# qq456cvb/CPPF2

Hardware: AMD Instinct MI355X
Metric: scenes/sec (1/2/4/8 GPU) at 4096 pts x 20k tuples; 5deg5cm match vs ref (higher is better)
Workload: dtype f32

## Files before the change

cppf2_amd/csrc/cppf_vote.hip:

```cpp
#include "cppf_common.h"
#include <mutex>

#define VC_THREADS 1024
#ifndef VC_SLAB_CELLS
#define VC_SLAB_CELLS 36864
#endif
#define VC_ARG_BLOCKS 32
#ifndef VC_MAX_LDS_ROTS
#define VC_MAX_LDS_ROTS 512
#endif
#define VC_TAB_LEN (2 * VC_MAX_LDS_ROTS + 4)
#define VC_LDS_WORDS (VC_SLAB_CELLS + 2 * VC_TAB_LEN + (VC_THREADS / 64) * 64)
#ifndef VC_MIN_SLAB_CELLS
#define VC_MIN_SLAB_CELLS 8192
#endif
#ifndef VC_MIN_WAVES
#define VC_MIN_WAVES 4
#endif
#define VC_FRAME_FLOATS 12
#define VC_WT_SCALE 256.0f
#ifndef VC_QUANTUM
#define VC_QUANTUM 4
#endif
#ifndef VC_ARC_MARGIN
// ... 546 lines not shown
    __syncthreads();
    const int item = s_item;
    if (item >= count) break;
    const uint32_t e = list[item / parts];
    const int b = (int)(e & 0xffffu), s = (int)(e >> 16);
    const CppfSceneGrid g = grids[b];
    vote_slab_item<true, WEIGHTED>(slab, tag, b, s, slab_cells, item % parts, parts, g, g.ncell, fr, total, tup_off, res, num_rots,
                                   cos_tab, sin_tab, grid, grid_off, cells_cap, slab_best, s_max, 1, part, tickets);
  }
}

__global__ __launch_bounds__(256) void vote_center_global_kernel(
    const float* __restrict__ pts, const int32_t* __restrict__ pt_off, const int32_t* __restrict__ idx, int k,
    const int32_t* __restrict__ tup_off, const float* __restrict__ tr, const float* __restrict__ vote_wt, float res,
    int num_rots, const float* __restrict__ cos_tab, const float* __restrict__ sin_tab,
    const CppfSceneGrid* __restrict__ grids, uint32_t* __restrict__ grid, const int64_t* __restrict__ grid_off,
    int64_t cells_cap) {
  const int b = blockIdx.y;
  const CppfSceneGrid g = grids[b];
  if ((int64_t)g.ncell > cells_cap || g.ncell <= 0) return;
  const float* p = pts + 3 * (int64_t)pt_off[b];
  const int t0 = tup_off[b], nt = tup_off[b + 1] - t0;
  uint32_t* gb = grid + (grid_off ? grid_off[b] : (int64_t)b * cells_cap);
  for (int t = blockIdx.x * blockDim.x + threadIdx.x; t < nt; t += gridDim.x * blockDim.x) {
    const int64_t row = (int64_t)(t0 + t);
    const VoteSetup v = vote_setup(p, idx[row * k], idx[row * k + 1], tr[row * 2], tr[row * 2 + 1], res);
    if (!v.ok) continue;
    const uint32_t wv = vote_weight(vote_wt, row);
    for (int r = 0; r < num_rots; ++r) {
      const int lin = vote_cell(v.cx, v.cy, v.cz, v.xx, v.xy, v.xz, v.yx, v.yy, v.yz, cos_tab[r], sin_tab[r],
                                g.c0[0], g.c0[1], g.c0[2], res, g.g[0], g.g[1], g.g[2]);
      if (lin >= 0) atomicAdd(&gb[lin], wv);
    }
  }
}

__global__ __launch_bounds__(256) void grid_argmax_partial_kernel(const uint32_t* __restrict__ grid,
                                                                  const int64_t* __restrict__ grid_off,
                                                                  int64_t cells_cap,
                                                                  const CppfSceneGrid* __restrict__ grids,
                                                                  SlabBest* __restrict__ partial, int s_max) {
  const int b = blockIdx.y;
  const int G = ((int64_t)grids[b].ncell <= cells_cap) ? grids[b].ncell : 0;
  const uint32_t* gb = grid + (grid_off ? grid_off[b] : (int64_t)b * cells_cap);
  const int per = (G + gridDim.x - 1) / gridDim.x;
  const int lo = blockIdx.x * per, hi = min(G, lo + per);
  uint32_t bv = 0;
  int64_t bi = INT64_MAX;
  for (int i = lo + threadIdx.x; i < hi; i += blockDim.x) argmax_combine(bv, bi, gb[i], (int64_t)i);
  wave_argmax(bv, bi);
  __shared__ uint32_t s_v[4];
  __shared__ int64_t s_i[4];
  if (wave_lane() == 0) { s_v[threadIdx.x >> 6] = bv; s_i[threadIdx.x >> 6] = bi; }
  __syncthreads();
  if (threadIdx.x == 0) {
    for (int w = 1; w < 4; ++w) argmax_combine(bv, bi, s_v[w], s_i[w]);
    SlabBest o; o.idx = bi; o.val = bv; o.pad = 0;
    partial[(int64_t)b * s_max + blockIdx.x] = o;
  }
}

__global__ __launch_bounds__(64) void grid_argmax_final_kernel(const SlabBest* __restrict__ partial, int s_max,
                                                               int fixed_parts, const int* __restrict__ ctl,
                                                               const CppfSceneGrid* __restrict__ grids,
                                                               int64_t cells_cap, double res,
                                                               int64_t* __restrict__ out_argmax,
                                                               uint32_t* __restrict__ out_peak,
                                                               double* __restrict__ out_world) {
  const int b = blockIdx.x;
  const CppfSceneGrid g = grids[b];
  const int G = ((int64_t)g.ncell <= cells_cap) ? g.ncell : 0;
  const int slab_cells = ctl ? ctl[3] : VC_SLAB_CELLS;
  const int parts = fixed_parts > 0 ? fixed_parts : (G + slab_cells - 1) / slab_cells;
  uint32_t bv = 0;
  int64_t bi = INT64_MAX;
  for (int i = threadIdx.x; i < parts; i += 64) {
    const SlabBest sb = partial[(int64_t)b * s_max + i];
    argmax_combine(bv, bi, sb.val, sb.idx);
  }
  wave_argmax(bv, bi);
  if (threadIdx.x == 0) {
    if (bi == INT64_MAX) bi = 0;
    out_argmax[b] = bi;
    if (out_peak) out_peak[b] = ((int64_t)g.ncell > cells_cap) ? 0xFFFFFFFFu : bv;
    if (out_world) {
      const int64_t gyz = (int64_t)g.g[1] * g.g[2];
      const int64_t ix = gyz > 0 ? bi / gyz : 0;
      const int64_t rem = gyz > 0 ? bi - ix * gyz : 0;
      const int64_t iy = g.g[2] > 0 ? rem / g.g[2] : 0;
      const int64_t iz = g.g[2] > 0 ? rem - iy * g.g[2] : 0;
      out_world[3 * b + 0] = (double)g.c0[0] + (double)ix * res;
      out_world[3 * b + 1] = (double)g.c0[1] + (double)iy * res;
      out_world[3 * b + 2] = (double)g.c0[2] + (double)iz * res;
    }
  }
}

__global__ __launch_bounds__(256) void grid_zero_kernel(uint32_t* __restrict__ grid,
                                                        const int64_t* __restrict__ grid_off, int64_t cells_cap,
                                                        const CppfSceneGrid* __restrict__ grids) {
  const int b = blockIdx.y;
  const int G = ((int64_t)grids[b].ncell <= cells_cap) ? grids[b].ncell : 0;
  uint32_t* gb = grid + (grid_off ? grid_off[b] : (int64_t)b * cells_cap);
  for (int i = blockIdx.x * blockDim.x + threadIdx.x; i < G; i += gridDim.x * blockDim.x) gb[i] = 0u;
}

static inline int64_t align_up(int64_t x, int64_t a) { return (x + a - 1) / a * a; }

static inline int vc_parts(int64_t cells_cap) {
  int64_t s_max = (cells_cap + VC_SLAB_CELLS - 1) / VC_SLAB_CELLS;
  if (s_max < VC_ARG_BLOCKS) s_max = VC_ARG_BLOCKS;
  return (int)s_max;
}

extern "C" int64_t cppf_vote_center_workspace_bytes(int B, int64_t cells_cap, int64_t total_tuples) {
  if (B <= 0 || cells_cap <= 0 || total_tuples < 0) return 0;
  return align_up((int64_t)B * vc_parts(cells_cap) * (int64_t)sizeof(SlabBest), 256) +
         align_up((int64_t)B * vc_parts(cells_cap) * 4 + 256, 256) + align_up((int64_t)B * vc_parts(cells_cap) * 4, 256) +
         align_up((int64_t)B * cells_cap * 4, 256) + align_up(total_tuples * VC_FRAME_FLOATS * 4, 256);
}

extern "C" int cppf_vote_center(int B, const float* pts, const int32_t* pt_off, const int32_t* idx, int k,
                                const int32_t* tup_off, int max_t, int64_t total_tuples, const float* tr,
                                const float* vote_wt, double res, int num_rots, const float* cos_tab, const float* sin_tab, const CppfSceneGrid* grids,
                                uint32_t* grid, const int64_t* grid_off, int64_t cells_cap, int mode,
                                void* workspace, int64_t workspace_bytes, int64_t* out_argmax, uint32_t* out_peak,
                                double* out_world, void* stream) {
  CPPF_CHECK_ARG(B > 0 && pts && pt_off && idx && tup_off && tr && cos_tab && sin_tab && grids && out_argmax);
  CPPF_CHECK_ARG(k >= 2 && num_rots > 0 && res > 0.0 && cells_cap > 0 && cells_cap <= 0x7fffffffLL);
  CPPF_CHECK_ARG(total_tuples >= 0 && max_t >= 0 && (int64_t)max_t <= total_tuples);
  CPPF_CHECK_ARG(workspace && workspace_bytes >= cppf_vote_center_workspace_bytes(B, cells_cap, total_tuples));
  CPPF_CHECK_ARG(grid == nullptr || grid_off != nullptr);
  hipStream_t st = (hipStream_t)stream;
  const int s_max_parts = vc_parts(cells_cap);
  SlabBest* best = (SlabBest*)workspace;
  char* wsp = (char*)workspace + align_up((int64_t)B * s_max_parts * sizeof(SlabBest), 256);
  int* ws_ctl = (int*)wsp;
  uint32_t* ws_list = (uint32_t*)(wsp + 256);
  wsp += align_up((int64_t)B * s_max_parts * 4 + 256, 256);
  int* ws_tickets = (int*)wsp;
  wsp += align_up((int64_t)B * s_max_parts * 4, 256);
  uint32_t* ws_grid = (uint32_t*)wsp;
  float* frames = (float*)(wsp + align_up((int64_t)B * cells_cap * 4, 256));
  const int s_max = (int)((cells_cap + VC_SLAB_CELLS - 1) / VC_SLAB_CELLS);
  const bool frames_only = (mode & CPPF_VC_FRAMES_ONLY) != 0, frames_ready = (mode & CPPF_VC_FRAMES_READY) != 0;
  const int mode_bits = mode;
  mode &= 0xff;
  if (mode == 0) mode = (s_max <= 64) ? 1 : 2;
  int exhaustive = 0;
  if (mode == 3) { mode = 1; exhaustive = 1; }
  const float res32 = (float)res;
  if (max_t <= 0) mode = 2;

  if (mode == 1) {
    int P = 1;
    const int64_t wgs = (int64_t)B * s_max;
    if (wgs < 256) {
      P = (int)((256 + wgs - 1) / wgs);
      const int pmax = (max_t + VC_THREADS - 1) / VC_THREADS;
      if (P > pmax) P = pmax;
      if (P < 1) P = 1;
    }
    const int lds_bytes = VC_LDS_WORDS * 4;
    static std::mutex cu_mutex;
    static int cu_count[64] = {0};
    int dev = 0;
    CPPF_HIP(hipGetDevice(&dev));
    const int dslot = dev & 63;
    {
      std::lock_guard<std::mutex> lock(cu_mutex);
      if (cu_count[dslot] == 0) {
        hipDeviceProp_t prop;
        CPPF_HIP(hipGetDeviceProperties(&prop, dev));
        const void* fns[] = {(const void*)vote_center_slab_kernel<true, false>, (const void*)vote_center_slab_kernel<true, true>,
                             (const void*)vote_center_slab_kernel<false, false>, (const void*)vote_center_slab_kernel<false, true>,
                             (const void*)vote_center_persist_kernel<false>, (const void*)vote_center_persist_kernel<true>};
        for (const void* f : fns) CPPF_HIP(hipFuncSetAttribute(f, hipFuncAttributeMaxDynamicSharedMemorySize, lds_bytes));
        cu_count[dslot] = prop.multiProcessorCount > 0 ? prop.multiProcessorCount : 256;
      }
    }
    const int num_cus = cu_count[dslot];
    const bool arcs = (exhaustive == 0) && s_max > 1 && num_rots <= VC_MAX_LDS_ROTS && num_rots >= 8;
    const bool persist = arcs && B <= 0xffff && s_max <= 0xffff && (mode_bits & 0x800) == 0;
    uint32_t* g_use = grid;
    const int64_t* goff_use = grid_off;
    if (P > 1 && !persist) {
      if (!g_use) { g_use = ws_grid; goff_use = nullptr; }
      hipLaunchKernelGGL(grid_zero_kernel, dim3(64, B), dim3(256), 0, st, g_use, goff_use, cells_cap, grids);
      CPPF_LAUNCH_CHECK();
    }
    if (persist) {
      const int pmax_t = (max_t + VC_THREADS - 1) / VC_THREADS;
      const int max_parts = (B <= 48) ? (pmax_t < 64 ? (pmax_t < 1 ? 1 : pmax_t) : 64) : 1;
      if (!frames_ready) {
        hipLaunchKernelGGL(vote_frames_kernel, dim3((max_t + 255) / 256, B), dim3(256), 0, st, pts, pt_off, idx, k,
                           tup_off, tr, vote_wt, res32, num_rots, total_tuples, frames);
        hipLaunchKernelGGL(vote_worklist_kernel, dim3(1), dim3(1024), 0, st, grids, B, cells_cap, s_max_parts, max_parts,
                           2 * num_cus, ws_list, ws_ctl);
        if (max_parts > 1) {
          hipLaunchKernelGGL(grid_zero_kernel, dim3(64, B), dim3(256), 0, st, ws_grid, (const int64_t*)nullptr, cells_cap,
                             grids);
          CPPF_HIP(hipMemsetAsync(ws_tickets, 0, (size_t)B * s_max_parts * 4, st));
        }
        CPPF_LAUNCH_CHECK();
      }
      if (frames_only) return CPPF_OK;
      if (vote_wt)
        hipLaunchKernelGGL(vote_center_persist_kernel<true>, dim3(num_cus), dim3(VC_THREADS), lds_bytes, st, frames,
                           total_tuples, tup_off, res32, num_rots, cos_tab, sin_tab, grids, grid, grid_off, cells_cap, best,
                           s_max_parts, ws_list, ws_ctl, max_parts > 1 ? ws_grid : (uint32_t*)nullptr, ws_tickets);
      else
        hipLaunchKernelGGL(vote_center_persist_kernel<false>, dim3(num_cus), dim3(VC_THREADS), lds_bytes, st, frames,
                           total_tuples, tup_off, res32, num_rots, cos_tab, sin_tab, grids, grid, grid_off, cells_cap, best,
                           s_max_parts, ws_list, ws_ctl, max_parts > 1 ? ws_grid : (uint32_t*)nullptr, ws_tickets);
      CPPF_LAUNCH_CHECK();
      hipLaunchKernelGGL(grid_argmax_final_kernel, dim3(B), dim3(64), 0, st, best, s_max_parts, 0, (const int*)ws_ctl, grids, cells_cap, res,
                         out_argmax, out_peak, out_world);
      CPPF_LAUNCH_CHECK();
      return CPPF_OK;
    }
    if (!frames_ready) {
      hipLaunchKernelGGL(vote_frames_kernel, dim3((max_t + 255) / 256, B), dim3(256), 0, st, pts, pt_off, idx, k,
                         tup_off, tr, vote_wt, res32, num_rots, total_tuples, frames);
      CPPF_LAUNCH_CHECK();
    }
    if (frames_only) return CPPF_OK;
    {
      const dim3 gr(B, P, s_max), bl(VC_THREADS);
#define VC_LAUNCH_SLAB(A, W)                                                                                          \
  hipLaunchKernelGGL((vote_center_slab_kernel<A, W>), gr, bl, lds_bytes, st, frames, total_tuples, tup_off, res32,       \
                     num_rots, cos_tab, sin_tab, grids, g_use, goff_use, cells_cap, best, s_max_parts, P)
      if (arcs) { if (vote_wt) VC_LAUNCH_SLAB(true, true); else VC_LAUNCH_SLAB(true, false); }
      else      { if (vote_wt) VC_LAUNCH_SLAB(false, true); else VC_LAUNCH_SLAB(false, false); }
#undef VC_LAUNCH_SLAB
    }
    CPPF_LAUNCH_CHECK();
    if (P == 1) {
      hipLaunchKernelGGL(grid_argmax_final_kernel, dim3(B), dim3(64), 0, st, best, s_max_parts, 0, (const int*)nullptr, grids, cells_cap,
                         res, out_argmax, out_peak, out_world);
    } else {
      hipLaunchKernelGGL(grid_argmax_partial_kernel, dim3(VC_ARG_BLOCKS, B), dim3(256), 0, st, g_use, goff_use,
                         cells_cap, grids, best, s_max_parts);
      hipLaunchKernelGGL(grid_argmax_final_kernel, dim3(B), dim3(64), 0, st, best, s_max_parts, VC_ARG_BLOCKS, (const int*)nullptr, grids,
                         cells_cap, res, out_argmax, out_peak, out_world);
    }
    CPPF_LAUNCH_CHECK();
    return CPPF_OK;
  }
  if (mode == 2) {
    uint32_t* g_use = grid ? grid : ws_grid;
    const int64_t* goff_use = grid ? grid_off : nullptr;
    hipLaunchKernelGGL(grid_zero_kernel, dim3(64, B), dim3(256), 0, st, g_use, goff_use, cells_cap, grids);
    CPPF_LAUNCH_CHECK();
    if (max_t > 0) {
      hipLaunchKernelGGL(vote_center_global_kernel, dim3((max_t + 255) / 256, B), dim3(256), 0, st, pts, pt_off, idx,
                         k, tup_off, tr, vote_wt, res32, num_rots, cos_tab, sin_tab, grids, g_use, goff_use, cells_cap);
      CPPF_LAUNCH_CHECK();
    }
    hipLaunchKernelGGL(grid_argmax_partial_kernel, dim3(VC_ARG_BLOCKS, B), dim3(256), 0, st, g_use, goff_use,
                       cells_cap, grids, best, s_max_parts);
    hipLaunchKernelGGL(grid_argmax_final_kernel, dim3(B), dim3(64), 0, st, best, s_max_parts, VC_ARG_BLOCKS, (const int*)nullptr, grids,
                       cells_cap, res, out_argmax, out_peak, out_world);
    CPPF_LAUNCH_CHECK();
    return CPPF_OK;
  }
  snprintf(g_cppf_err, sizeof(g_cppf_err), "cppf_vote_center: unknown mode %d", mode);
  return CPPF_EINVAL;
}

#ifndef BV_THREADS
#define BV_THREADS 1024
#endif

__device__ __forceinline__ int block_scan_flag(bool flag, int* s_wave, int* total) {
  const unsigned long long m = __ballot(flag);
  const int lane = wave_lane(), w = threadIdx.x >> 6;
  const int within = __popcll(m & ((1ull << lane) - 1ull));
  if (lane == 0) s_wave[w] = __popcll(m);
  __syncthreads();
  int base = 0, tot = 0;
  for (int i = 0; i < BV_THREADS / 64; ++i) {
    const int c = s_wave[i];
    if (i < w) base += c;
    tot += c;
  }
  __syncthreads();
  *total = tot;
  return base + within;
}

template <typename KeyFn>
__device__ uint32_t radix_select_keys(KeyFn key, int n, int kth, uint32_t* s_hist , int* s_misc ,
                                      int* n_le) {
  uint32_t prefix = 0;
  int remaining = kth;
  int below = 0;
  const int shifts[3] = {21, 10, 0};
  const int widths[3] = {11, 11, 10};
  uint32_t mask_fixed = 0;
  for (int pass = 0; pass < 3; ++pass) {
    const int sh = shifts[pass], nbins = 1 << widths[pass];
    for (int i = threadIdx.x; i < nbins; i += blockDim.x) s_hist[i] = 0;
    __syncthreads();
    for (int i = threadIdx.x; i < n; i += blockDim.x) {
      const uint32_t bits = key(i);
      if ((bits & mask_fixed) == prefix) atomicAdd(&s_hist[(bits >> sh) & (nbins - 1)], 1u);
    }
    __syncthreads();
    if (threadIdx.x < 64) {
      const int per = nbins / 64;
      uint32_t sum = 0;
      for (int j = 0; j < per; ++j) sum += s_hist[threadIdx.x * per + j];
      uint32_t incl = sum;
#pragma unroll
      for (int off = 1; off < 64; off <<= 1) {
        const uint32_t o = __shfl_up(incl, off);
        if ((int)threadIdx.x >= off) incl += o;
      }
      const uint32_t excl = incl - sum;
      if ((uint32_t)remaining >= excl && (uint32_t)remaining < incl) {
        uint32_t run = excl;
        for (int j = 0; j < per; ++j) {
          const uint32_t c = s_hist[threadIdx.x * per + j];
          if ((uint32_t)remaining < run + c) {
            s_misc[0] = threadIdx.x * per + j;
            s_misc[1] = (int)run;
            s_misc[2] = (int)c;
            break;
          }
          run += c;
        }
      }
    }
    __syncthreads();
    const int bin = s_misc[0];
    below += s_misc[1];
    remaining -= s_misc[1];
    prefix |= ((uint32_t)bin) << sh;
    mask_fixed |= ((uint32_t)(nbins - 1)) << sh;
    if (pass == 2) *n_le = below + s_misc[2];
    __syncthreads();
  }
  return prefix;
}

__device__ uint32_t radix_select(const float* __restrict__ v, int n, int kth, uint32_t* s_hist, int* s_misc,
                                 int* n_le) {
  return radix_select_keys([v](int i) { return __float_as_uint(v[i]); }, n, kth, s_hist, s_misc, n_le);
}

__device__ __forceinline__ uint32_t float_key(float f) {
  const uint32_t u = __float_as_uint(f);
  return (u & 0x80000000u) ? ~u : (u | 0x80000000u);
}
__device__ __forceinline__ float key_float(uint32_t k) {
  return __uint_as_float((k & 0x80000000u) ? (k & 0x7fffffffu) : ~k);
}

__global__ __launch_bounds__(256) void backvote_errs_kernel(const float* __restrict__ pts,
                                                            const int32_t* __restrict__ pt_off,
                                                            const int32_t* __restrict__ idx, int k,
                                                            const int32_t* __restrict__ tup_off,
                                                            const float* __restrict__ tr,
                                                            const double* __restrict__ centers, Axes9 axes,
                                                            float* __restrict__ errs) {
  const int b = blockIdx.y;
  const float* p = pts + 3 * (int64_t)pt_off[b];
  const int t0 = tup_off[b], nt = tup_off[b + 1] - t0;
  const double cx = centers[3 * b], cy = centers[3 * b + 1], cz = centers[3 * b + 2];
  for (int t = blockIdx.x * 256 + threadIdx.x; t < nt; t += gridDim.x * 256) {
    const int64_t row = (int64_t)(t0 + t);
    const float* a = p + 3 * (int64_t)idx[row * k];
    const float* bb = p + 3 * (int64_t)idx[row * k + 1];
    float tb[2];
    target_pair(a[0], a[1], a[2], bb[0], bb[1], bb[2], cx, cy, cz, axes.a, tb, nullptr);
    const float d0 = tr[row * 2] - tb[0], d1 = tr[row * 2 + 1] - tb[1];
    errs[row] = __builtin_sqrtf(d0 * d0 + d1 * d1);
  }
}

__global__ __launch_bounds__(BV_THREADS) void backvote_kernel(
    const float* __restrict__ pts, const int32_t* __restrict__ pt_off, const int32_t* __restrict__ idx, int k,
    const int32_t* __restrict__ tup_off, const float* __restrict__ tr, const double* __restrict__ centers,
    Axes9 axes, const int32_t* __restrict__ kidx, const float* __restrict__ gammas, double margin, int num_rots,
    uint8_t* __restrict__ mask, int32_t* __restrict__ kept_tuple, int32_t* __restrict__ kept_count,
    double* __restrict__ kept_wt, int32_t* __restrict__ kept_row0, float* __restrict__ errs,
    float* __restrict__ thr_out, int32_t* __restrict__ hits) {
  __shared__ uint32_t s_hist[2048];
  __shared__ int s_misc[4];
  __shared__ int s_wave[BV_THREADS / 64];
  __shared__ float s_f[BV_THREADS / 64];
  const int b = blockIdx.x;
  const int p0 = pt_off[b];
  const float* p = pts + 3 * (int64_t)p0;
  const int t0 = tup_off[b], nt = tup_off[b + 1] - t0;
  float* e = errs + t0;
  if (nt <= 0) {
    if (threadIdx.x == 0) { kept_count[b] = 0; if (thr_out) thr_out[b] = NAN; }
    return;
  }
  int kq = kidx[b];
  if (kq > nt - 1) kq = nt - 1;
  const float gamma = gammas[b];
  int n_le = 0;
  const uint32_t bits_lo = radix_select(e, nt, kq, s_hist, s_misc, &n_le);
  const float v_lo = __uint_as_float(bits_lo);
  float v_hi = v_lo;
  if (kq + 1 <= nt - 1 && kq + 1 >= n_le) {
    uint32_t mn = 0xffffffffu;
    for (int i = threadIdx.x; i < nt; i += BV_THREADS) {
      const uint32_t bits = __float_as_uint(e[i]);
      if (bits > bits_lo && bits < mn) mn = bits;
    }
#pragma unroll
    for (int off = 32; off > 0; off >>= 1) mn = min(mn, (uint32_t)__shfl_xor((int)mn, off));
    if (wave_lane() == 0) s_hist[threadIdx.x >> 6] = mn;
    __syncthreads();
    if (threadIdx.x == 0) {
      for (int w = 1; w < BV_THREADS / 64; ++w) mn = min(mn, s_hist[w]);
      s_hist[64] = mn;
    }
    __syncthreads();
    v_hi = __uint_as_float(s_hist[64]);
    __syncthreads();
  }
  const float diff = v_hi - v_lo;
  float thr = v_lo + diff * gamma;
  if (gamma >= 0.5f) thr = v_hi - diff * (1.0f - gamma);
  if (threadIdx.x == 0 && thr_out) thr_out[b] = thr;
  int kept = 0;
  for (int base = 0; base < nt; base += BV_THREADS) {
    const int t = base + threadIdx.x;
    const bool keep = (t < nt) && (e[t] < thr);
    if (t < nt) mask[t0 + t] = keep ? 1 : 0;
    int tot;
    const int pos = block_scan_flag(keep, s_wave, &tot);
    if (keep) kept_tuple[t0 + kept + pos] = t;
    kept += tot;
  }
  if (threadIdx.x == 0) kept_count[b] = kept;
  __syncthreads();
  int32_t* h = hits + p0;
  for (int j = threadIdx.x; j < kept; j += BV_THREADS) {
    const int64_t row = (int64_t)(t0 + kept_tuple[t0 + j]);
    atomicAdd(&h[idx[row * k]], 1);
    atomicAdd(&h[idx[row * k + 1]], 1);
  }
  __threadfence();
  __syncthreads();
  int hmax = 0;
  for (int j = threadIdx.x; j < kept; j += BV_THREADS) {
    const int64_t row = (int64_t)(t0 + kept_tuple[t0 + j]);
    hmax = max(hmax, __hip_atomic_load(&h[idx[row * k]], __ATOMIC_RELAXED, __HIP_MEMORY_SCOPE_AGENT));
    hmax = max(hmax, __hip_atomic_load(&h[idx[row * k + 1]], __ATOMIC_RELAXED, __HIP_MEMORY_SCOPE_AGENT));
  }
#pragma unroll
  for (int off = 32; off > 0; off >>= 1) hmax = max(hmax, __shfl_xor(hmax, off));
  if (wave_lane() == 0) s_wave[threadIdx.x >> 6] = hmax;
  __syncthreads();
  hmax = 0;
  for (int w = 0; w < BV_THREADS / 64; ++w) hmax = max(hmax, s_wave[w]);
  __syncthreads();
  const double dmax = (double)hmax;
  int rank = 0;
  for (int base = 0; base < kept; base += BV_THREADS) {
    const int j = base + threadIdx.x;
    bool valid = false;
    if (j < kept) {
      const int64_t row = (int64_t)(t0 + kept_tuple[t0 + j]);
      const int i0 = idx[row * k], i1 = idx[row * k + 1];
      const double w0 = (double)__hip_atomic_load(&h[i0], __ATOMIC_RELAXED, __HIP_MEMORY_SCOPE_AGENT) / dmax;
      const double w1 = (double)__hip_atomic_load(&h[i1], __ATOMIC_RELAXED, __HIP_MEMORY_SCOPE_AGENT) / dmax;
      kept_wt[t0 + j] = (w0 + w1) + margin;
      const float dx = p[3 * i0] - p[3 * i1], dy = p[3 * i0 + 1] - p[3 * i1 + 1], dz = p[3 * i0 + 2] - p[3 * i1 + 2];
      valid = norm3_fused(dx, dy, dz) > 1e-7f;
    }
    int tot;
    const int pos = block_scan_flag(valid, s_wave, &tot);
    if (j < kept) kept_row0[t0 + j] = valid ? (rank + pos) * num_rots : -1;
    rank += tot;
  }
  (void)s_f;
}

extern "C" int64_t cppf_backvote_workspace_bytes(int64_t total_points, int B) {
  (void)B;
  return align_up(total_points * 4, 256);
}

extern "C" int cppf_backvote_filter(int B, const float* pts, const int32_t* pt_off, const int32_t* idx, int k,
                                    const int32_t* tup_off, const float* tr, const double* centers,
                                    const double* h_axes, const int32_t* kidx, const float* gammas,
                                    double imp_wt_margin, int num_rots, uint8_t* mask, int32_t* kept_tuple,
                                    int32_t* kept_count, double* kept_wt, int32_t* kept_row0, float* back_errs,
                                    float* thr, void* workspace, int64_t workspace_bytes, void* stream) {
  CPPF_CHECK_ARG(B > 0 && pts && pt_off && idx && tup_off && tr && centers && h_axes && kidx && gammas);
  CPPF_CHECK_ARG(mask && kept_tuple && kept_count && kept_wt && kept_row0 && back_errs);
  CPPF_CHECK_ARG(workspace && workspace_bytes > 0);
  Axes9 ax;
  for (int i = 0; i < 9; ++i) ax.a[i] = h_axes[i];
  CPPF_HIP(hipMemsetAsync(workspace, 0, (size_t)workspace_bytes, (hipStream_t)stream));
  hipLaunchKernelGGL(backvote_errs_kernel, dim3(B >= 32 ? 16 : 64, B), dim3(256), 0, (hipStream_t)stream, pts, pt_off,
                     idx, k, tup_off, tr, centers, ax, back_errs);
  CPPF_LAUNCH_CHECK();
  hipLaunchKernelGGL(backvote_kernel, dim3(B), dim3(BV_THREADS), 0, (hipStream_t)stream, pts, pt_off, idx, k, tup_off,
                     tr, centers, ax, kidx, gammas, imp_wt_margin, num_rots, mask, kept_tuple, kept_count, kept_wt,
                     kept_row0, back_errs, thr, (int32_t*)workspace);
  CPPF_LAUNCH_CHECK();
  return CPPF_OK;
}

#define RB_THREADS 256
#define RB_MAX_CAND 1024

struct RotCand {
  float x, y, z;
  int slot;
  double inv_wt;
};

__device__ __forceinline__ void rot_candidate(const PairFrame& f, float tn, float cs, float sn, float& ox, float& oy,
                                              float& oz) {
  const float den = fmaxf(f.nco, 1e-7f);
  const float xx = f.cox / den, xy = f.coy / den, xz = f.coz / den;
  const float yx = cross_term(xy, f.uz, xz, f.uy);
  const float yy = cross_term(xz, f.ux, xx, f.uz);
  const float yz = cross_term(xx, f.uy, xy, f.ux);
  const float offx = cs * xx + sn * yx, offy = cs * xy + sn * yy, offz = cs * xz + sn * yz;
  const float sg = (tn > 0.0f) ? 1.0f : -1.0f;
  const float ux = tn * offx + sg * f.ux, uy = tn * offy + sg * f.uy, uz = tn * offz + sg * f.uz;
  const float n = fmaxf(norm3_fused(ux, uy, uz), 1e-7f);
  ox = ux / n; oy = uy / n; oz = uz / n;
}

__global__ __launch_bounds__(RB_THREADS) void rot_bins_dense_kernel(
    const float* __restrict__ pts, const int32_t* __restrict__ pt_off, const int32_t* __restrict__ idx, int k,
    const int32_t* __restrict__ tup_off, const float* __restrict__ rot, int rot_col,
    const int32_t* __restrict__ kept_tuple, const int32_t* __restrict__ kept_count,
    const double* __restrict__ kept_wt, const int32_t* __restrict__ kept_row0, int pairs_per_block, int num_rots,
    const float* __restrict__ cos_tab, const float* __restrict__ sin_tab, const float* __restrict__ sphere, int S,
    float cos_thr, int bmm_size, int max_chunks, double* __restrict__ sums ) {
  __shared__ RotCand s_c[RB_MAX_CAND];
  __shared__ int s_cb;
  const int b = blockIdx.y;
  const int kept = kept_count[b];
  const int j0 = blockIdx.x * pairs_per_block;
  if (j0 >= kept) return;
  const int npairs = min(pairs_per_block, kept - j0);
  const int ncand = npairs * num_rots;
  const int t0 = tup_off[b];
  const float* p = pts + 3 * (int64_t)pt_off[b];
  if (threadIdx.x == 0) s_cb = 0x7fffffff;
  __syncthreads();
  for (int c = threadIdx.x; c < ncand; c += RB_THREADS) {
    const int pj = c / num_rots, r = c - pj * num_rots;
    const int j = j0 + pj;
    const int row0 = kept_row0[t0 + j];
    RotCand rc;
    rc.slot = -1; rc.x = rc.y = rc.z = 0.0f; rc.inv_wt = 0.0;
    if (row0 >= 0) {
      const int64_t row = (int64_t)(t0 + kept_tuple[t0 + j]);
      const PairFrame f = pair_frame(p, idx[row * k], idx[row * k + 1]);
      const float tn = tanf(rot[row * 3 + rot_col]);
      rot_candidate(f, tn, cos_tab[r], sin_tab[r], rc.x, rc.y, rc.z);
      rc.slot = (row0 + r) / bmm_size;
      rc.inv_wt = 1.0 / kept_wt[t0 + j];
      atomicMin(&s_cb, rc.slot);
    }
    s_c[c] = rc;
  }
  __syncthreads();
  const int cb = s_cb;
  if (cb == 0x7fffffff) return;
  double* out = sums + ((int64_t)b * max_chunks) * S;
  for (int s = threadIdx.x; s < S; s += RB_THREADS) {
    const float bx = sphere[3 * s], by = sphere[3 * s + 1], bz = sphere[3 * s + 2];
    double acc0 = 0.0, acc1 = 0.0;
    for (int c = 0; c < ncand; ++c) {
      const RotCand rc = s_c[c];
      if (rc.slot < 0) continue;
      const float d = fmaf(rc.z, bz, fmaf(rc.y, by, rc.x * bx));
      const double w = (d > cos_thr) ? rc.inv_wt : 0.0;
      if (rc.slot == cb) acc0 += w; else acc1 += w;
    }
    if (acc0 != 0.0) atomicAdd(&out[(int64_t)cb * S + s], acc0);
    if (acc1 != 0.0) atomicAdd(&out[(int64_t)(cb + 1) * S + s], acc1);
  }
}

#define RW_THREADS 256
#define RL_K 8
struct RwFrame {
  float xx, xy, xz, yx, yy, yz, ux, uy, uz;
  float tn[2];
  int row0;
  double inv_wt;
};

template <int NAX>
__global__ __launch_bounds__(RW_THREADS) void rot_bins_lut_kernel(
    const float* __restrict__ pts, const int32_t* __restrict__ pt_off, const int32_t* __restrict__ idx, int k,
    const int32_t* __restrict__ tup_off, const float* __restrict__ rot, int rot_col0, int rot_col1,
    const int32_t* __restrict__ kept_tuple, const int32_t* __restrict__ kept_count,
    const double* __restrict__ kept_wt, const int32_t* __restrict__ kept_row0, int rows_per_block, int sub_blocks,
    int max_pairs, int num_rots, const float* __restrict__ cos_tab, const float* __restrict__ sin_tab,
    const float* __restrict__ sphere, int S, float cos_thr, const int4* __restrict__ lut, int lut_rows, int lut_cols,
    int bmm_size, double* __restrict__ partial ) {
  extern __shared__ __attribute__((aligned(16))) char smem[];
  float4* s_sph = (float4*)smem;
  unsigned long long* s_acc = (unsigned long long*)(smem + (size_t)S * 16);
  float2* s_trig = (float2*)(s_acc + (size_t)NAX * S);
  RwFrame* s_fr = (RwFrame*)(s_trig + num_rots);
  int* s_list = (int*)(s_fr + max_pairs);
  __shared__ int s_n;
  __shared__ unsigned long long s_maxw;
  const int b = blockIdx.y;
  const int chunk = blockIdx.x / sub_blocks, sub = blockIdx.x - chunk * sub_blocks;
  const int64_t lo64 = (int64_t)chunk * bmm_size + (int64_t)sub * rows_per_block;
  const int64_t hi64 = min(lo64 + rows_per_block, (int64_t)(chunk + 1) * bmm_size);
  const int kept = kept_count[b];
  const int t0 = tup_off[b];
  double* out = partial + ((int64_t)b * gridDim.x + blockIdx.x) * NAX * S;
  if (threadIdx.x == 0) {
    s_n = 0;
    s_maxw = 0;
  }
  __syncthreads();
  if (lo64 < (int64_t)kept * num_rots) {
    const int lo = (int)lo64, hi = (int)min(hi64, (int64_t)kept * num_rots);
    for (int j = threadIdx.x; j < kept; j += RW_THREADS) {
      const int row0 = kept_row0[t0 + j];
      if (row0 >= 0 && row0 < hi && row0 + num_rots > lo) {
        const int pos = atomicAdd(&s_n, 1);
        if (pos < max_pairs) s_list[pos] = j;
      }
    }
  }
  __syncthreads();
  const int npairs = min(s_n, max_pairs);
  if (npairs == 0) {
    for (int i = threadIdx.x; i < NAX * S; i += RW_THREADS) out[i] = 0.0;
    return;
  }
  const int lo = (int)lo64, hi = (int)hi64;
  const float* p = pts + 3 * (int64_t)pt_off[b];
  for (int i = threadIdx.x; i < S; i += RW_THREADS)
    s_sph[i] = make_float4(sphere[3 * i], sphere[3 * i + 1], sphere[3 * i + 2], 0.0f);
  for (int i = threadIdx.x; i < NAX * S; i += RW_THREADS) s_acc[i] = 0ull;
  for (int i = threadIdx.x; i < num_rots; i += RW_THREADS) s_trig[i] = make_float2(cos_tab[i], sin_tab[i]);
  for (int i = threadIdx.x; i < npairs; i += RW_THREADS) {
    const int j = s_list[i];
    const int64_t row = (int64_t)(t0 + kept_tuple[t0 + j]);
    const PairFrame f = pair_frame(p, idx[row * k], idx[row * k + 1]);
    RwFrame fr;
    const float den = fmaxf(f.nco, 1e-7f);
    fr.xx = f.cox / den; fr.xy = f.coy / den; fr.xz = f.coz / den;
    fr.yx = cross_term(fr.xy, f.uz, fr.xz, f.uy);
    fr.yy = cross_term(fr.xz, f.ux, fr.xx, f.uz);
    fr.yz = cross_term(fr.xx, f.uy, fr.xy, f.ux);
    fr.ux = f.ux; fr.uy = f.uy; fr.uz = f.uz;
    fr.tn[0] = tanf(rot[row * 3 + rot_col0]);
    fr.tn[1] = (NAX > 1) ? tanf(rot[row * 3 + rot_col1]) : 0.0f;
    fr.row0 = kept_row0[t0 + j];
    fr.inv_wt = 1.0 / kept_wt[t0 + j];
    s_fr[i] = fr;
    if (fr.inv_wt > 0.0 && fr.inv_wt < 1e300) atomicMax(&s_maxw, (unsigned long long)__double_as_longlong(fr.inv_wt));
  }
  __syncthreads();
  int fx_e;
  {
    const double bound = (double)rows_per_block * fmax(__longlong_as_double((long long)s_maxw), 1e-300);
    int eb;
    frexp(bound, &eb);
    fx_e = 62 - eb;
  }
  for (int i = threadIdx.x; i < npairs; i += RW_THREADS) {
    const double w = s_fr[i].inv_wt;
    const unsigned long long q = (w > 0.0 && w < 1e300) ? (unsigned long long)__double2ll_rn(ldexp(w, fx_e)) : 0ull;
    s_fr[i].inv_wt = __longlong_as_double((long long)q);
  }
  __syncthreads();
  const float row_scale = 0.5f * (float)lut_rows, col_scale = (float)lut_cols * 0.15915494309189535f;
  const int ncand = npairs * num_rots;
  const int dq = RW_THREADS / num_rots, dr = RW_THREADS - dq * num_rots;
  int pj = (int)threadIdx.x / num_rots, r = (int)threadIdx.x - pj * num_rots;
  for (int c = threadIdx.x; c < ncand; c += RW_THREADS) {
    const RwFrame fr = s_fr[pj];
    const int row = fr.row0 + r;
    const float2 t = s_trig[r];
    pj += dq; r += dr;
    if (r >= num_rots) { r -= num_rots; ++pj; }
    if (row < lo || row >= hi) continue;
    const float cs = t.x, sn = t.y;
    const float offx = cs * fr.xx + sn * fr.yx, offy = cs * fr.xy + sn * fr.yy, offz = cs * fr.xz + sn * fr.yz;
#pragma unroll
    for (int a = 0; a < NAX; ++a) {
      const float tn = fr.tn[a];
      const float sg = (tn > 0.0f) ? 1.0f : -1.0f;
      const float ux = tn * offx + sg * fr.ux, uy = tn * offy + sg * fr.uy, uz = tn * offz + sg * fr.uz;
      const float nn = fmaxf(norm3_fused(ux, uy, uz), 1e-7f);
      const float x = ux / nn, y = uy / nn, z = uz / nn;
      if (!(y == y) || !(x == x) || !(z == z)) continue;
      float phi = atan2_poly(z, x);
      phi += (phi < 0.0f) ? 6.2831853071795865f : 0.0f;
      int ci = (int)((1.0f - y) * row_scale), cj = (int)(phi * col_scale);
      ci = min(max(ci, 0), lut_rows - 1);
      cj = min(max(cj, 0), lut_cols - 1);
      const int4 e = lut[ci * lut_cols + cj];
      const int ids[4] = {e.x, e.y, e.z, e.w};
#pragma unroll
      for (int h = 0; h < 4; ++h) {
#pragma unroll
        for (int lo16 = 0; lo16 < 2; ++lo16) {
          const int s = lo16 ? (ids[h] >> 16) : (int)(short)(ids[h] & 0xffff);
          if (s >= 0) {
            const float4 q = s_sph[s];
            const float d = fmaf(z, q.z, fmaf(y, q.y, x * q.x));
            if (d > cos_thr) atomicAdd(&s_acc[a * S + s], (unsigned long long)__double_as_longlong(fr.inv_wt));
          }
        }
      }
    }
  }
  __syncthreads();
  for (int i = threadIdx.x; i < NAX * S; i += RW_THREADS) out[i] = ldexp((double)s_acc[i], -fx_e);
}

__global__ __launch_bounds__(1024) void rot_bins_fold_kernel(const double* __restrict__ partial, int nblk,
                                                            int sub_blocks, int nax, int S, int B,
                                                            float* __restrict__ counts, int32_t* __restrict__ top_idx,
                                                            float* __restrict__ top_count) {
  const int b = blockIdx.x, a = blockIdx.y;
  const double* part = partial + ((int64_t)b * nblk * nax + a) * S;
  const int64_t bstride = (int64_t)nax * S;
  float best = -INFINITY;
  int besti = 0x7fffffff;
  for (int s = threadIdx.x; s < S; s += blockDim.x) {
    float c = 0.0f;
    for (int i0 = 0; i0 < nblk; i0 += sub_blocks) {
      double acc = 0.0;
      for (int k0 = 0; k0 < sub_blocks; k0 += 8) {
        double v[8];
#pragma unroll
        for (int k = 0; k < 8; ++k) v[k] = (k0 + k < sub_blocks) ? part[(i0 + k0 + k) * bstride + s] : 0.0;
#pragma unroll
        for (int k = 0; k < 8; ++k) acc += v[k];
      }
      c = (float)((double)c + acc);
    }
    counts[((int64_t)a * B + b) * S + s] = c;
    if (c > best || (c == best && s < besti)) { best = c; besti = s; }
  }
#pragma unroll
  for (int off = 32; off > 0; off >>= 1) {
    const float ob = __shfl_xor(best, off);
    const int oi = __shfl_xor(besti, off);
    if (ob > best || (ob == best && oi < besti)) { best = ob; besti = oi; }
  }
  __shared__ float s_b[16];
  __shared__ int s_i[16];
  if (wave_lane() == 0) { s_b[threadIdx.x >> 6] = best; s_i[threadIdx.x >> 6] = besti; }
  __syncthreads();
  if (threadIdx.x == 0) {
    for (int w = 1; w < (int)(blockDim.x >> 6); ++w)
      if (s_b[w] > best || (s_b[w] == best && s_i[w] < besti)) { best = s_b[w]; besti = s_i[w]; }
    if (besti == 0x7fffffff) besti = 0;
    if (top_idx) top_idx[(int64_t)a * B + b] = besti;
    if (top_count) top_count[(int64_t)a * B + b] = best;
  }
}

__global__ __launch_bounds__(256) void rot_bins_final_kernel(const double* __restrict__ sums, int S, int max_chunks,
                                                             float* __restrict__ counts, int32_t* __restrict__ top_idx,
                                                             float* __restrict__ top_count) {
  const int b = blockIdx.x;
  const double* in = sums + ((int64_t)b * max_chunks) * S;
  float best = -INFINITY;
  int besti = 0x7fffffff;
  for (int s = threadIdx.x; s < S; s += blockDim.x) {
    float c = 0.0f;
    for (int ch = 0; ch < max_chunks; ++ch) c = (float)((double)c + in[(int64_t)ch * S + s]);
    counts[(int64_t)b * S + s] = c;
    if (c > best || (c == best && s < besti)) { best = c; besti = s; }
  }
#pragma unroll
  for (int off = 32; off > 0; off >>= 1) {
    const float ob = __shfl_xor(best, off);
    const int oi = __shfl_xor(besti, off);
    if (ob > best || (ob == best && oi < besti)) { best = ob; besti = oi; }
  }
  __shared__ float s_b[4];
  __shared__ int s_i[4];
  if (wave_lane() == 0) { s_b[threadIdx.x >> 6] = best; s_i[threadIdx.x >> 6] = besti; }
  __syncthreads();
  if (threadIdx.x == 0) {
    for (int w = 1; w < 4; ++w)
      if (s_b[w] > best || (s_b[w] == best && s_i[w] < besti)) { best = s_b[w]; besti = s_i[w]; }
    if (besti == 0x7fffffff) besti = 0;
    if (top_idx) top_idx[b] = besti;
    if (top_count) top_count[b] = best;
  }
}

static inline int rb_max_chunks(int max_kept, int num_rots, int bmm_size) {
  const int64_t rows = (int64_t)max_kept * num_rots;
  return (int)((rows + bmm_size - 1) / bmm_size) + 1;
}

struct RwPlan {
  int nchunks, sub, rpb, nblk, max_pairs;
};

static inline RwPlan rw_plan(int B, int max_kept, int num_rots, int bmm_size) {
  RwPlan pl;
  const int64_t rows = (int64_t)(max_kept > 0 ? max_kept : 1) * num_rots;
  pl.nchunks = (int)((rows + bmm_size - 1) / bmm_size);
  const int64_t target = (int64_t)(B >= 16 ? 160 : 32) * num_rots;
  pl.sub = (target >= bmm_size) ? 1 : (int)((bmm_size + target - 1) / target);
  pl.rpb = (bmm_size + pl.sub - 1) / pl.sub;
  pl.nblk = pl.nchunks * pl.sub;
  pl.max_pairs = pl.rpb / num_rots + 2;
  return pl;
}

extern "C" int64_t cppf_rot_bins_workspace_bytes(int B, int S, int max_kept, int num_rots, int bmm_size) {
  if (B <= 0 || S <= 0 || max_kept < 0 || num_rots <= 0 || bmm_size <= 0) return 0;
  const int64_t dense = align_up((int64_t)B * rb_max_chunks(max_kept, num_rots, bmm_size) * S * 8, 256);
  const RwPlan pl = rw_plan(B, max_kept, num_rots, bmm_size);
  const int64_t window = align_up((int64_t)B * pl.nblk * 2 * S * 8, 256);
  return dense > window ? dense : window;
}

static int rot_bins_dense_launch(int B, const float* pts, const int32_t* pt_off, const int32_t* idx, int k,
                                 const int32_t* tup_off, const float* rot, int rot_col, const int32_t* kept_tuple,
                                 const int32_t* kept_count, const double* kept_wt, const int32_t* kept_row0,
                                 int max_kept, int num_rots, const float* cos_tab, const float* sin_tab,
                                 const float* sphere, int S, float cos_thr, int bmm_size, float* counts,
                                 int32_t* top_idx, float* top_count, void* workspace, hipStream_t st) {
  const int max_chunks = rb_max_chunks(max_kept, num_rots, bmm_size);
  double* sums = (double*)workspace;
  CPPF_HIP(hipMemsetAsync(sums, 0, (size_t)B * max_chunks * S * 8, st));
  if (max_kept > 0) {
    int ppb = RB_MAX_CAND / num_rots;
    if (ppb > 4) ppb = 4;
    if (ppb < 1) ppb = 1;
    if ((int64_t)ppb * num_rots > bmm_size) ppb = bmm_size / num_rots;
    const int blocks = (max_kept + ppb - 1) / ppb;
    hipLaunchKernelGGL(rot_bins_dense_kernel, dim3(blocks, B), dim3(RB_THREADS), 0, st, pts, pt_off, idx, k, tup_off,
                       rot, rot_col, kept_tuple, kept_count, kept_wt, kept_row0, ppb, num_rots, cos_tab, sin_tab,
                       sphere, S, cos_thr, bmm_size, max_chunks, sums);
    CPPF_LAUNCH_CHECK();
  }
  hipLaunchKernelGGL(rot_bins_final_kernel, dim3(B), dim3(256), 0, st, sums, S, max_chunks, counts, top_idx,
                     top_count);
  CPPF_LAUNCH_CHECK();
  return CPPF_OK;
}

static int rot_bins_impl(int nax, int B, const float* pts, const int32_t* pt_off, const int32_t* idx, int k,
                         const int32_t* tup_off, const float* rot, int rot_col0, int rot_col1,
                         const int32_t* kept_tuple, const int32_t* kept_count, const double* kept_wt,
                         const int32_t* kept_row0, int max_kept, int num_rots, const float* cos_tab,
                         const float* sin_tab, const float* sphere, int S, float cos_thr, int bmm_size,
                         const int16_t* bin_lut, int lut_rows, int lut_cols, float* counts, int32_t* top_idx,
                         float* top_count, void* workspace, int64_t workspace_bytes, void* stream) {
  CPPF_CHECK_ARG(B > 0 && pts && pt_off && idx && tup_off && rot && kept_tuple && kept_count && kept_wt && kept_row0);
  CPPF_CHECK_ARG(cos_tab && sin_tab && sphere && counts);
  CPPF_CHECK_ARG(rot_col0 >= 0 && rot_col0 < 3 && rot_col1 >= 0 && rot_col1 < 3);
  CPPF_CHECK_ARG(S > 0 && num_rots > 0 && num_rots <= RB_MAX_CAND && bmm_size > 0);
  CPPF_CHECK_ARG(bin_lut == nullptr || (lut_rows > 0 && lut_cols > 0 && S <= 32767));
  CPPF_CHECK_ARG((int64_t)max_kept * num_rots < 0x7fffffffLL);
  CPPF_CHECK_ARG(workspace && workspace_bytes >= cppf_rot_bins_workspace_bytes(B, S, max_kept, num_rots, bmm_size));
  hipStream_t st = (hipStream_t)stream;
  if (num_rots > bmm_size) {
    snprintf(g_cppf_err, sizeof(g_cppf_err), "cppf_rot_bins: bmm_size %d < num_rots %d unsupported", bmm_size, num_rots);
    return CPPF_EUNSUPPORTED;
  }
  const RwPlan pl = rw_plan(B, max_kept, num_rots, bmm_size);
  const size_t lut_need = (size_t)S * 16 + (size_t)nax * S * 8 + (size_t)num_rots * 8 +
                          (size_t)pl.max_pairs * (sizeof(RwFrame) + 4);
  const size_t lut_lds = lut_need;
  if (bin_lut && lut_need <= 64000 && max_kept > 0) {
    double* partial = (double*)workspace;
    if (nax == 2)
      hipLaunchKernelGGL(rot_bins_lut_kernel<2>, dim3(pl.nblk, B), dim3(RW_THREADS), lut_lds, st, pts, pt_off, idx, k,
                         tup_off, rot, rot_col0, rot_col1, kept_tuple, kept_count, kept_wt, kept_row0, pl.rpb, pl.sub,
                         pl.max_pairs, num_rots, cos_tab, sin_tab, sphere, S, cos_thr, (const int4*)bin_lut, lut_rows,
                         lut_cols, bmm_size, partial);
    else
      hipLaunchKernelGGL(rot_bins_lut_kernel<1>, dim3(pl.nblk, B), dim3(RW_THREADS), lut_lds, st, pts, pt_off, idx, k,
                         tup_off, rot, rot_col0, rot_col1, kept_tuple, kept_count, kept_wt, kept_row0, pl.rpb, pl.sub,
                         pl.max_pairs, num_rots, cos_tab, sin_tab, sphere, S, cos_thr, (const int4*)bin_lut, lut_rows,
                         lut_cols, bmm_size, partial);
    CPPF_LAUNCH_CHECK();
    const int fold_threads = S >= 1024 ? 1024 : ((S + 63) / 64) * 64;
    hipLaunchKernelGGL(rot_bins_fold_kernel, dim3(B, nax), dim3(fold_threads), 0, st, partial, pl.nblk, pl.sub, nax, S, B, counts,
                       top_idx, top_count);
    CPPF_LAUNCH_CHECK();
    return CPPF_OK;
  }
  for (int a = 0; a < nax; ++a) {
    const int rc = rot_bins_dense_launch(B, pts, pt_off, idx, k, tup_off, rot, a ? rot_col1 : rot_col0, kept_tuple,
                                         kept_count, kept_wt, kept_row0, max_kept, num_rots, cos_tab, sin_tab, sphere, S,
                                         cos_thr, bmm_size, counts + (int64_t)a * B * S,
                                         top_idx ? top_idx + (int64_t)a * B : nullptr,
                                         top_count ? top_count + (int64_t)a * B : nullptr, workspace, st);
    if (rc != CPPF_OK) return rc;
  }
  return CPPF_OK;
}

extern "C" int cppf_rot_bins(int B, const float* pts, const int32_t* pt_off, const int32_t* idx, int k,
                             const int32_t* tup_off, const float* rot, int rot_col, const int32_t* kept_tuple,
                             const int32_t* kept_count, const double* kept_wt, const int32_t* kept_row0, int max_kept,
                             int num_rots, const float* cos_tab, const float* sin_tab, const float* sphere, int S,
                             float cos_thr, int bmm_size, const int16_t* bin_lut, int lut_rows, int lut_cols,
                             float* counts, int32_t* top_idx, float* top_count, void* workspace,
                             int64_t workspace_bytes, void* stream) {
  return rot_bins_impl(1, B, pts, pt_off, idx, k, tup_off, rot, rot_col, rot_col, kept_tuple, kept_count, kept_wt,
                       kept_row0, max_kept, num_rots, cos_tab, sin_tab, sphere, S, cos_thr, bmm_size, bin_lut, lut_rows,
                       lut_cols, counts, top_idx, top_count, workspace, workspace_bytes, stream);
}

extern "C" int cppf_rot_bins2(int B, const float* pts, const int32_t* pt_off, const int32_t* idx, int k,
                              const int32_t* tup_off, const float* rot, int rot_col0, int rot_col1,
                              const int32_t* kept_tuple, const int32_t* kept_count, const double* kept_wt,
                              const int32_t* kept_row0, int max_kept, int num_rots, const float* cos_tab,
                              const float* sin_tab, const float* sphere, int S, float cos_thr, int bmm_size,
                              const int16_t* bin_lut, int lut_rows, int lut_cols, float* counts, int32_t* top_idx,
                              float* top_count, void* workspace, int64_t workspace_bytes, void* stream) {
  return rot_bins_impl(2, B, pts, pt_off, idx, k, tup_off, rot, rot_col0, rot_col1, kept_tuple, kept_count, kept_wt,
                       kept_row0, max_kept, num_rots, cos_tab, sin_tab, sphere, S, cos_thr, bmm_size, bin_lut, lut_rows,
                       lut_cols, counts, top_idx, top_count, workspace, workspace_bytes, stream);
}

__global__ __launch_bounds__(1024) void vr_scan_kernel(const float* __restrict__ pts, const int32_t* __restrict__ idx,
                                                       int k, int T, uint8_t* __restrict__ valid,
                                                       int32_t* __restrict__ rank, int32_t* __restrict__ n_valid) {
  __shared__ int s_wave[BV_THREADS / 64];
  int base_rank = 0;
  for (int base = 0; base < T; base += BV_THREADS) {
    const int t = base + threadIdx.x;
    bool v = false;
    if (t < T) {
      const int i0 = idx[(int64_t)t * k], i1 = idx[(int64_t)t * k + 1];
      v = norm3_fused(pts[3 * i0] - pts[3 * i1], pts[3 * i0 + 1] - pts[3 * i1 + 1],
                      pts[3 * i0 + 2] - pts[3 * i1 + 2]) > 1e-7f;
      valid[t] = v ? 1 : 0;
    }
    int tot;
    const int pos = block_scan_flag(v, s_wave, &tot);
    if (t < T) rank[t] = v ? base_rank + pos : -1;
    base_rank += tot;
  }
  if (threadIdx.x == 0) *n_valid = base_rank;
}

__global__ __launch_bounds__(256) void vr_emit_kernel(const float* __restrict__ pts, const int32_t* __restrict__ idx,
                                                      int k, int T, const float* __restrict__ angle, int num_rots,
                                                      const float* __restrict__ cos_tab,
                                                      const float* __restrict__ sin_tab,
                                                      const int32_t* __restrict__ rank, float* __restrict__ up) {
  const int64_t total = (int64_t)T * num_rots;
  for (int64_t c = (int64_t)blockIdx.x * blockDim.x + threadIdx.x; c < total; c += (int64_t)gridDim.x * blockDim.x) {
    const int t = (int)(c / num_rots), r = (int)(c - (int64_t)t * num_rots);
    const int rk = rank[t];
    if (rk < 0) continue;
    const PairFrame f = pair_frame(pts, idx[(int64_t)t * k], idx[(int64_t)t * k + 1]);
    float x, y, z;
    rot_candidate(f, tanf(angle[t]), cos_tab[r], sin_tab[r], x, y, z);
    float* o = up + ((int64_t)rk * num_rots + r) * 3;
    o[0] = x; o[1] = y; o[2] = z;
  }
}

extern "C" int cppf_vote_rotation(const float* pts, int n_points, const int32_t* idx, int k, int T,
                                  const float* rot_angle, int num_rots, const float* cos_tab, const float* sin_tab,
                                  float* up, uint8_t* valid, int32_t* n_valid, void* workspace,
                                  int64_t workspace_bytes, void* stream) {
  CPPF_CHECK_ARG(pts && idx && rot_angle && cos_tab && sin_tab && up && valid && n_valid && workspace);
  CPPF_CHECK_ARG(n_points > 0 && k >= 2 && T >= 0 && num_rots > 0 && workspace_bytes >= (int64_t)T * 4);
  hipStream_t st = (hipStream_t)stream;
  int32_t* rank = (int32_t*)workspace;
  hipLaunchKernelGGL(vr_scan_kernel, dim3(1), dim3(BV_THREADS), 0, st, pts, idx, k, T, valid, rank, n_valid);
  CPPF_LAUNCH_CHECK();
  if (T > 0) {
    const int64_t blocks = ((int64_t)T * num_rots + 255) / 256;
    hipLaunchKernelGGL(vr_emit_kernel, dim3((unsigned)(blocks < 16384 ? blocks : 16384)), dim3(256), 0, st, pts, idx, k,
                       T, rot_angle, num_rots, cos_tab, sin_tab, rank, up);
    CPPF_LAUNCH_CHECK();
  }
  return CPPF_OK;
}

#define SC_ROWS 512
__global__ __launch_bounds__(256) void sphere_counts_kernel(const float* __restrict__ cand, int64_t M,
                                                            const double* __restrict__ wt,
                                                            const float* __restrict__ sphere, int S, float cos_thr,
                                                            int bmm_size, int blocks_per_chunk,
                                                            double* __restrict__ sums) {
  __shared__ float s_x[SC_ROWS], s_y[SC_ROWS], s_z[SC_ROWS];
  __shared__ double s_w[SC_ROWS];
  const int chunk = blockIdx.x / blocks_per_chunk, sub = blockIdx.x - chunk * blocks_per_chunk;
  const int64_t c_lo = (int64_t)chunk * bmm_size;
  const int64_t c_hi = (c_lo + bmm_size < M) ? c_lo + bmm_size : M;
  const int64_t lo = c_lo + (int64_t)sub * SC_ROWS;
  if (lo >= c_hi) return;
  const int n = (int)((c_hi - lo < SC_ROWS) ? c_hi - lo : SC_ROWS);
  for (int i = threadIdx.x; i < n; i += blockDim.x) {
    s_x[i] = cand[(lo + i) * 3]; s_y[i] = cand[(lo + i) * 3 + 1]; s_z[i] = cand[(lo + i) * 3 + 2];
    s_w[i] = wt ? 1.0 / wt[lo + i] : 1.0;
  }
  __syncthreads();
  for (int s = threadIdx.x; s < S; s += blockDim.x) {
    const float bx = sphere[3 * s], by = sphere[3 * s + 1], bz = sphere[3 * s + 2];
    double acc = 0.0;
    for (int i = 0; i < n; ++i) {
      const float d = fmaf(s_z[i], bz, fmaf(s_y[i], by, s_x[i] * bx));
      acc += (d > cos_thr) ? s_w[i] : 0.0;
    }
// ... 164 lines not shown
```

Baseline: 5156.

## Batch loads in radix select, prefetch errors, and double rot-bin block size

The radix-select histogram and min-scan loops now load eight keys per thread before processing them, so several memory loads are in flight at once. The threshold/keep loop prefetches the next error value one iteration ahead. The LUT rot-bin kernel grows from 256 to 512 threads per block, and its per-axis LUT gathers are split from the sphere-dot accumulation so the loads can overlap. The costs are higher register pressure and possibly lower occupancy; the block-size change also alters how candidates map to threads and the shared-memory atomic contention pattern.

Result: no change. 5163, median of 6 (+0.1%).

```diff
diff --git a/cppf2_amd/csrc/cppf_vote.hip b/cppf2_amd/csrc/cppf_vote.hip
--- a/cppf2_amd/csrc/cppf_vote.hip
+++ b/cppf2_amd/csrc/cppf_vote.hip
@@ -872,9 +872,13 @@
     const int sh = shifts[pass], nbins = 1 << widths[pass];
     for (int i = threadIdx.x; i < nbins; i += blockDim.x) s_hist[i] = 0;
     __syncthreads();
-    for (int i = threadIdx.x; i < n; i += blockDim.x) {
-      const uint32_t bits = key(i);
-      if ((bits & mask_fixed) == prefix) atomicAdd(&s_hist[(bits >> sh) & (nbins - 1)], 1u);
+    for (int i0 = threadIdx.x; i0 < n; i0 += 8 * blockDim.x) {
+      uint32_t bits[8];
+#pragma unroll
+      for (int u = 0; u < 8; ++u) bits[u] = (i0 + u * (int)blockDim.x < n) ? key(i0 + u * (int)blockDim.x) : 0u;
+#pragma unroll
+      for (int u = 0; u < 8; ++u)
+        if (i0 + u * (int)blockDim.x < n && (bits[u] & mask_fixed) == prefix) atomicAdd(&s_hist[(bits[u] >> sh) & (nbins - 1)], 1u);
     }
     __syncthreads();
     if (threadIdx.x < 64) {
@@ -978,9 +982,13 @@
   float v_hi = v_lo;
   if (kq + 1 <= nt - 1 && kq + 1 >= n_le) {
     uint32_t mn = 0xffffffffu;
-    for (int i = threadIdx.x; i < nt; i += BV_THREADS) {
-      const uint32_t bits = __float_as_uint(e[i]);
-      if (bits > bits_lo && bits < mn) mn = bits;
+    for (int i0 = threadIdx.x; i0 < nt; i0 += 8 * BV_THREADS) {
+      uint32_t bits[8];
+#pragma unroll
+      for (int u = 0; u < 8; ++u) bits[u] = (i0 + u * BV_THREADS < nt) ? __float_as_uint(e[i0 + u * BV_THREADS]) : 0u;
+#pragma unroll
+      for (int u = 0; u < 8; ++u)
+        if (bits[u] > bits_lo && bits[u] < mn) mn = bits[u];
     }
 #pragma unroll
     for (int off = 32; off > 0; off >>= 1) mn = min(mn, (uint32_t)__shfl_xor((int)mn, off));
@@ -999,9 +1007,12 @@
   if (gamma >= 0.5f) thr = v_hi - diff * (1.0f - gamma);
   if (threadIdx.x == 0 && thr_out) thr_out[b] = thr;
   int kept = 0;
+  float e_next = ((int)threadIdx.x < nt) ? e[threadIdx.x] : 0.0f;
   for (int base = 0; base < nt; base += BV_THREADS) {
     const int t = base + threadIdx.x;
-    const bool keep = (t < nt) && (e[t] < thr);
+    const float e_t = e_next;
+    e_next = (t + BV_THREADS < nt) ? e[t + BV_THREADS] : 0.0f;
+    const bool keep = (t < nt) && (e_t < thr);
     if (t < nt) mask[t0 + t] = keep ? 1 : 0;
     int tot;
     const int pos = block_scan_flag(keep, s_wave, &tot);
@@ -1158,7 +1169,7 @@
   }
 }
 
-#define RW_THREADS 256
+#define RW_THREADS 512
 #define RL_K 8
 struct RwFrame {
   float xx, xy, xz, yx, yy, yz, ux, uy, uz;
@@ -1263,21 +1274,27 @@
     if (row < lo || row >= hi) continue;
     const float cs = t.x, sn = t.y;
     const float offx = cs * fr.xx + sn * fr.yx, offy = cs * fr.xy + sn * fr.yy, offz = cs * fr.xz + sn * fr.yz;
+    float x[NAX], y[NAX], z[NAX];
+    int4 e[NAX];
 #pragma unroll
     for (int a = 0; a < NAX; ++a) {
       const float tn = fr.tn[a];
       const float sg = (tn > 0.0f) ? 1.0f : -1.0f;
       const float ux = tn * offx + sg * fr.ux, uy = tn * offy + sg * fr.uy, uz = tn * offz + sg * fr.uz;
       const float nn = fmaxf(norm3_fused(ux, uy, uz), 1e-7f);
-      const float x = ux / nn, y = uy / nn, z = uz / nn;
-      if (!(y == y) || !(x == x) || !(z == z)) continue;
-      float phi = atan2_poly(z, x);
+      x[a] = ux / nn; y[a] = uy / nn; z[a] = uz / nn;
+      e[a] = make_int4(-1, -1, -1, -1);
+      if (!(y[a] == y[a]) || !(x[a] == x[a]) || !(z[a] == z[a])) continue;
+      float phi = atan2_poly(z[a], x[a]);
       phi += (phi < 0.0f) ? 6.2831853071795865f : 0.0f;
-      int ci = (int)((1.0f - y) * row_scale), cj = (int)(phi * col_scale);
+      int ci = (int)((1.0f - y[a]) * row_scale), cj = (int)(phi * col_scale);
       ci = min(max(ci, 0), lut_rows - 1);
       cj = min(max(cj, 0), lut_cols - 1);
-      const int4 e = lut[ci * lut_cols + cj];
-      const int ids[4] = {e.x, e.y, e.z, e.w};
+      e[a] = lut[ci * lut_cols + cj];
+    }
+#pragma unroll
+    for (int a = 0; a < NAX; ++a) {
+      const int ids[4] = {e[a].x, e[a].y, e[a].z, e[a].w};
 #pragma unroll
       for (int h = 0; h < 4; ++h) {
 #pragma unroll
@@ -1285,7 +1302,7 @@
           const int s = lo16 ? (ids[h] >> 16) : (int)(short)(ids[h] & 0xffff);
           if (s >= 0) {
             const float4 q = s_sph[s];
-            const float d = fmaf(z, q.z, fmaf(y, q.y, x * q.x));
+            const float d = fmaf(z[a], q.z, fmaf(y[a], q.y, x[a] * q.x));
             if (d > cos_thr) atomicAdd(&s_acc[a * S + s], (unsigned long long)__double_as_longlong(fr.inv_wt));
           }
         }
```
